# marl-book/codebase

Measured on NVIDIA H100. Metric: env-steps/sec, higher is better.
Workload: dtype f32

## Files before the change

codebase_b200/csrc/dqn.cu:

```cuda
#include "learner.cuh"
#include "dqn_heads.cuh"
#include "retms.cuh"
#include "qmix.cuh"
#include "gru.cuh"
#include <math.h>
#include <stdlib.h>
#include <string.h>
#include <vector>

namespace marl {

__global__ void replay_sample_kernel(uint64_t seed, uint64_t update_idx, int batch, int n_valid, int32_t* idx) {
  const int i = blockIdx.x * blockDim.x + threadIdx.x;
  pdl_wait();
  pdl_launch_dependents();
  if (i >= batch) return;
  const u32x4 b = philox4x32_10((uint32_t)update_idx, (uint32_t)(update_idx >> 32), (uint32_t)(i >> 2), 0u, (uint32_t)seed, (uint32_t)(seed >> 32) ^ kTagSample);
  idx[i] = (int32_t)bounded(pick(b, i & 3), (uint32_t)n_valid);
}

struct ColTdParams {
  const float* q; const float* tq;
  TrajView traj; const int32_t* idx; int B, A; float gamma; int double_q;
  int C, G;
// ... 477 lines not shown
    } else {
      qmix_mix_fn(hl, 0)<<<qb, kQmWarps * 32, qm_smem_bytes(h->ql), st>>>(qp, h->mix_img, h->mix_img_tgt);
    }
    const int want = h->mix_wgrad_tiles ? kQmixChunks : 2 * h->n_sm;
    const int chunk_len = (((Sn + want - 1) / want) + 31) & ~31, chunks = (Sn + chunk_len - 1) / chunk_len;
    if (h->mix_wgrad_tiles) {
      qmix_wgrad_kernel<<<dim3(h->mix_n_tiles, chunks), 256, 0, st>>>(h->mix_rec, Sn, h->mix_tiles, chunk_len, h->mix_part, n);
    } else {
      for (int round = 0; round * kQmMicroPerRound < h->mix_n_micro; ++round)
        qmix_wgrad2_kernel<<<chunks, 256, (size_t)(h->ql.R + 2) * kQmP * sizeof(float), st>>>(h->mix_rec, Sn, h->ql.R, h->mix_micro, h->mix_n_micro, round, chunk_len, h->mix_part, n);
    }
    qmix_reduce_kernel<<<(n + 255) / 256, 256, 0, st>>>(h->mix_part, chunks, n, h->mix_grad, qp.loss_part, qb);
    MARL_CUDA_TRY(cudaGetLastError());
    n_loss_parts += qb;
    tp.td_agent_stride = batch * T;
    return MARL_OK;
  }
  const bool vdn = h->hp.mixer == 1;
  ColTdParams cp; memset(&cp, 0, sizeof(cp));
  cp.q = h->q_all; cp.tq = h->tq; cp.traj = src.traj; cp.idx = src.idx; cp.B = batch; cp.A = h->ns.out;
  cp.gamma = h->hp.gamma; cp.double_q = h->hp.double_q; cp.huber = h->huber; cp.C = vdn ? 1 : h->ns.n_agents; cp.G = vdn ? h->ns.n_agents : 1;
  cp.td = h->td; cp.loss_part = loss_part;
  const int blocks = (cp.C * batch * T + 255) / 256;
  if (h->td_lambda_on) {
    cp.ret = h->ret; cp.chosen = h->chosen; cp.boot = h->boot; cp.stat_per_b = vdn;
    if (h->standardise) { cp.ret_ms = h->ret_ms; cp.n_stat = h->n_stat; }
    col_td_kernel<3><<<blocks, 256, 0, st>>>(cp);
    if (int rc = dqn_td_lambda(h, src, cp.C, cp.G, batch, st)) return rc;
    if (h->standardise) {
      RetMsParams rp; rp.ret = h->ret; rp.part = h->ret_part; rp.ret_ms = h->ret_ms; rp.count = h->ret_count; rp.T = T;
      if (vdn) { rp.N = batch; rp.P = 1; } else { rp.N = cp.C; rp.P = batch; }
      MARL_CUDA_TRY(ret_ms_step(rp, st));
    }
    col_td_kernel<2><<<blocks, 256, 0, st>>>(cp);
  } else if (h->standardise) {
    cp.ret_ms = h->ret_ms; cp.n_stat = h->n_stat; cp.stat_per_b = vdn; cp.ret = h->ret; cp.chosen = h->chosen;
    col_td_kernel<1><<<blocks, 256, 0, st>>>(cp);
    RetMsParams rp; rp.ret = h->ret; rp.part = h->ret_part; rp.ret_ms = h->ret_ms; rp.count = h->ret_count; rp.T = T;
    if (vdn) { rp.N = batch; rp.P = 1; } else { rp.N = cp.C; rp.P = batch; }
    MARL_CUDA_TRY(ret_ms_step(rp, st));
    col_td_kernel<2><<<blocks, 256, 0, st>>>(cp);
  } else {
    col_td_kernel<0><<<blocks, 256, 0, st>>>(cp);
  }
  MARL_CUDA_TRY(cudaGetLastError());
  n_loss_parts += blocks;
  tp.td_agent_stride = vdn ? 0 : batch * T;
  return MARL_OK;
}

static bool dqn_tc_train(const marl_dqn* h) { return !h->rnn && tc_backward_enabled() && h->ns.in < kMaxObsDim && h->image != nullptr; }

static int dqn_tc_prepare(marl_dqn* h, TcBuffers& tb, cudaStream_t st) {
  if (!h->tc_h2) {
    const size_t rows = (size_t)h->ns.n_agents * h->max_batch * (h->max_T + 1), F = sizeof(float);
    if (int rc = alloc_buffers(h, "marl_dqn_update", {{&h->tc_h2, rows * kHidden * F},
                                                      {&h->tc_rec, rows * 32  * F}, {&h->tc_x, rows * ((h->ns.in + 7) / 8 * 8) * F},
                                                      {&h->image_bwd, ((size_t)h->ns.n_nets * tc_bwd_image_bytes() / 4 + 4) * F}}))
      return rc;
  }
  if (!h->image_current || !h->bwd_image_current) {
    if (int rc = launch_pack_weights(h->theta, h->ns.lay, h->ns.n_nets, h->image, st, h->image_bwd)) return rc;
    h->image_current = h->bwd_image_current = true;
  }
  tb.image = h->image; tb.bwd_image = h->image_bwd; tb.h2 = h->tc_h2; tb.rec = h->tc_rec; tb.x = h->tc_x; tb.rows = (size_t)h->ns.n_agents * h->max_batch * (h->max_T + 1);
  return MARL_OK;
}

static int dqn_train_pass(marl_dqn* h, const TrainParams& tp, cudaEvent_t* between, bool& tc, cudaStream_t st) {
  tc = false;
  if (h->rnn) {
    GruBwdParams bp; memset(&bp, 0, sizeof(bp));
    bp.plan = tp.plan; bp.traj = tp.src.traj; bp.idx = tp.src.idx; bp.B = tp.plan.units_per_agent; bp.theta = h->theta; bp.lay = h->gl; bp.save = h->gru_save;
    bp.td = tp.td_ext; bp.td_agent_stride = tp.td_agent_stride; bp.src = tp.src; bp.scratch = h->scratch; bp.scratch_pitch = h->scratch_pitch;
    return launch_gru_backward(bp, st);
  }
  if (!dqn_tc_train(h)) return launch_train(tp, kHeadDqn, st);
  TcBuffers tb;
  if (int rc = dqn_tc_prepare(h, tb, st)) return rc;
  tc = true;
  if (int rc = launch_tc_dqn_forward(tp, tb, nullptr, nullptr, nullptr, st)) return rc;
  if (between) MARL_CUDA_TRY(cudaEventRecord(between[0], st));
  return launch_tc_dqn_backward(tp, tb, st, between ? between[1] : nullptr);
}

static int dqn_fused_pass(marl_dqn* h, const RowPlan& plan, const RowSource& src, int batch, TrainParams& tp, int& n_loss_parts, cudaEvent_t* ev,
                          cudaStream_t st) {
  TcBuffers tb;
  if (int rc = dqn_tc_prepare(h, tb, st)) return rc;
  if (!h->tgt_image_current) {
    if (int rc = launch_pack_weights(h->theta_tgt, h->ns.lay, h->ns.n_nets, h->image_tgt, st)) return rc;
    h->tgt_image_current = true;
  }
  if (ev) MARL_CUDA_TRY(cudaEventRecord(ev[0], st));
  if (int rc = launch_tc_dqn_forward(tp, tb, h->image_tgt, h->tq, dqn_external_head(h) ? h->q_all : nullptr, st)) return rc;
  if (ev) MARL_CUDA_TRY(cudaEventRecord(ev[1], st));
  if (int rc = dqn_td_head(h, plan, src, batch, tp, n_loss_parts, false, st)) return rc;
  if (int rc = launch_tc_dqn_backward(tp, tb, st, ev ? ev[2] : nullptr)) return rc;
  if (ev) { MARL_CUDA_TRY(cudaEventRecord(ev[3], st)); h->ev_used += 1; h->ev_split = true; }
  return MARL_OK;
}

static int dqn_grads(marl_dqn* h, const marl_traj_view* traj, const int32_t* episode_idx, int32_t batch, void* stream, ReduceParams* rp_out) {
  MARL_REQUIRE(h && traj && episode_idx, "marl_dqn_update_grads: NULL argument");
  MARL_REQUIRE(batch >= 1 && batch <= h->max_batch, "marl_dqn_update_grads: batch %d exceeds max_batch %d", batch, h->max_batch);
  MARL_REQUIRE(traj->T >= 1 && traj->T <= h->max_T, "marl_dqn_update_grads: T %d exceeds max_T %d", traj->T, h->max_T);
  MARL_REQUIRE(traj->n_agents == h->ns.n_agents && traj->obs_dim == h->ns.in, "marl_dqn_update_grads: trajectory shape mismatch");
  MARL_REQUIRE(h->hp.mixer != 2 || h->mix != nullptr, "marl_dqn_update: QMIX needs marl_dqn_qmix_init first");
  MARL_REQUIRE(h->hp.mixer == 0 || !h->standardise || batch == h->n_stat, "marl_dqn_update: %s's standardise_returns keeps one statistic per batch entry (the "
               "reference's reshape(-1, B)): batch %d must stay at max_batch %d", h->hp.mixer == 2 ? "QMIX" : "VDN", batch, h->n_stat);
  MARL_CUDA_TRY(cudaSetDevice(h->device));
  cudaStream_t st = (cudaStream_t)stream;
  const RowPlan plan = h->rnn ? make_plan(h->ns, batch, 1, h->n_sm, kGruSeqs) : episode_plan(h->ns, batch, traj->T, h->n_sm);
  const RowSource src = episode_rows(traj, episode_idx, h->ns.n_agents, h->ns.in);
  cudaEvent_t* ev = h->timing && h->ev_used < kTimingPairs ? &h->ev[4 * h->ev_used] : nullptr;
  TrainParams tp; memset(&tp, 0, sizeof(tp));
  tp.plan = plan; tp.src = src; tp.theta = h->theta; tp.lay = h->ns.lay; tp.tq = h->tq;
  tp.gamma = h->hp.gamma; tp.double_q = h->hp.double_q; tp.huber = h->huber; tp.scratch = h->scratch; tp.scratch_pitch = h->scratch_pitch; tp.loss_part = h->loss_part;
// ... 247 lines not shown
```

codebase_b200/csrc/learner.cuh:

```cuda
#pragma once
#include "mlp.cuh"
#include "traj.cuh"
#include <string.h>

namespace marl {

constexpr int kMaxObsDim = 32;
constexpr int kMaxInDim = 128;

struct RowPlan {
  int n_nets;
  int cta_begin[MARL_MAX_AGENTS + 1];
  int slot_begin[MARL_MAX_AGENTS + 1];
  int slot_agent[MARL_MAX_AGENTS];
  int unit_rows;
  int units_per_agent;
};

enum RowMode {
  kRowsDense = 0,
  kRowsEpisode = 1,
  kRowsEpisodeJoint = 2,
  kRowsDenseJoint = 3
};
// ... 190 lines not shown
  p.n_nets = ns.n_nets; p.unit_rows = unit_rows; p.units_per_agent = units_per_agent;
  int s = 0;
  for (int k = 0; k < ns.n_nets; ++k) {
    p.slot_begin[k] = s;
    for (int a = 0; a < ns.n_agents; ++a) if (ns.agent_net[a] == k) p.slot_agent[s++] = a;
  }
  p.slot_begin[ns.n_nets] = s;
  long long total = (long long)ns.n_agents * units_per_agent;
  int c = 0;
  for (int k = 0; k < ns.n_nets; ++k) {
    const long long units = (long long)(p.slot_begin[k + 1] - p.slot_begin[k]) * units_per_agent;
    long long want = (long long)n_cta_max * units / (total > 0 ? total : 1);
    const long long cap = (units + min_units - 1) / min_units;
    if (want > cap) want = cap;
    if (want < 1) want = 1;
    p.cta_begin[k] = c;
    c += (int)want;
  }
  p.cta_begin[ns.n_nets] = c;
  return p;
}

inline RowPlan episode_plan(const NetSet& ns, int episodes, int T, int n_cta_max) {
  const int min_units = (64 + T) / (T + 1) > 0 ? (64 + T) / (T + 1) : 1;
  return make_plan(ns, episodes, T + 1, n_cta_max, min_units);
}

inline RowSource dense_rows(const float* obs, int E, int N, int D, bool joint = false) {
  RowSource s; memset(&s, 0, sizeof(s));
  s.mode = joint ? kRowsDenseJoint : kRowsDense; s.dense = obs; s.E = E; s.N = N; s.D = D;
  if (joint) s.joint = obs;
  return s;
}

inline RowSource episode_rows(const marl_traj_view* t, const int32_t* idx, int N, int D) {
  RowSource s; memset(&s, 0, sizeof(s));
  s.mode = kRowsEpisode; s.traj = traj_view(t); s.idx = idx; s.N = N; s.D = D;
  return s;
}

inline int launch_forward(const NetSet& ns, const RowPlan& plan, const RowSource& src, const float* theta, float* out, cudaStream_t st) {
  FwdParams fp; fp.plan = plan; fp.src = src; fp.theta = theta; fp.lay = ns.lay; fp.out = out;
  return launch_mlp_forward(fp, st);
}

size_t tc_image_bytes();
int tc_forward_init();
size_t tc_bwd_image_bytes();
int launch_pack_weights(const float* theta, const NetLayout& lay, int n_nets, uint8_t* image, cudaStream_t st, uint8_t* bwd_image = nullptr);
int launch_tc_forward(const FwdParams& p, const uint8_t* images, cudaStream_t st);
struct TcBuffers {
  uint8_t* image; uint8_t* bwd_image;
  float* h2;
  float* rec;
  float* x;
  size_t rows;
};
int tc_train_init();
int launch_tc_dqn_forward(const TrainParams& tp, const TcBuffers& buf, const uint8_t* tgt_images, float* tq_out, float* q_out, cudaStream_t st);
int launch_tc_dqn_backward(const TrainParams& tp, const TcBuffers& buf, cudaStream_t st, cudaEvent_t after_dh1 = nullptr);

inline int forward_any(const NetSet& ns, const RowPlan& plan, const RowSource& src, const float* theta, uint8_t* image, float* out, cudaStream_t st,
                       bool image_is_current = false) {
  if (tc_forward_enabled() && image != nullptr && ns.in <= kMaxObsDim && ns.lay.H == kHidden) {
    if (!image_is_current)
      if (int rc = launch_pack_weights(theta, ns.lay, ns.n_nets, image, st)) return rc;
    FwdParams fp; fp.plan = plan; fp.src = src; fp.theta = theta; fp.lay = ns.lay; fp.out = out;
    return launch_tc_forward(fp, image, st);
  }
  return launch_forward(ns, plan, src, theta, out, st);
}

inline int check_mlp_cfg(const marl_mlp_cfg* cfg, const char* who, int max_in) {
  MARL_REQUIRE(cfg != nullptr, "%s: NULL network config", who);
  MARL_REQUIRE(cfg->n_agents >= 1 && cfg->n_agents <= MARL_MAX_AGENTS, "%s: n_agents out of range", who);
  MARL_REQUIRE(cfg->n_nets >= 1 && cfg->n_nets <= cfg->n_agents, "%s: n_nets out of range", who);
  MARL_REQUIRE(cfg->hidden >= 1 && cfg->hidden <= kHidden, "%s: hidden width %d not supported (layers = [H, H], 1 <= H <= %d)", who, cfg->hidden, kHidden);
  MARL_REQUIRE(cfg->in_dim >= 1 && cfg->in_dim <= max_in, "%s: obs dim %d not supported (1..%d)", who, cfg->in_dim, max_in);
  MARL_REQUIRE(cfg->out_dim >= 1 && cfg->out_dim <= kOutPad, "%s: output width %d not supported (1..%d)", who, cfg->out_dim, kOutPad);
  for (int a = 0; a < cfg->n_agents; ++a) MARL_REQUIRE(cfg->agent_net[a] >= 0 && cfg->agent_net[a] < cfg->n_nets, "%s: agent_net[%d] out of range", who, a);
  return MARL_OK;
}

inline NetSet to_netset(const marl_mlp_cfg* cfg) {
  NetSet ns; ns.n_agents = cfg->n_agents; ns.n_nets = cfg->n_nets; ns.in = cfg->in_dim; ns.out = cfg->out_dim;
  memcpy(ns.agent_net, cfg->agent_net, sizeof(int) * MARL_MAX_AGENTS);
  ns.lay = NetLayout::make(cfg->in_dim, cfg->out_dim, cfg->hidden);
  return ns;
}

struct LearnerHandle : BufferOwner {
  int device = 0, n_sm = 148;
  int64_t n_params = 0;
  int scratch_pitch = 0;
  float *theta = nullptr, *theta_tgt = nullptr, *m = nullptr, *v = nullptr, *grad = nullptr, *scratch = nullptr, *loss_part = nullptr;
  int32_t* idx = nullptr;
  uint8_t* image = nullptr;
  marl_optimizer opt = {};
  bool opt_stepped = false;
  int standardise = 0, n_stat = 0; float* ret_ms = nullptr; double *ret_count = nullptr, *ret_part = nullptr;
};

template <typename H, typename HP>
int open_learner(int device, const HP& hp, H** out) {
  if (int rc = check_device(device)) return rc;
  H* h = new H();
  h->hp = hp; h->device = device;
  cudaDeviceProp prop; cudaGetDeviceProperties(&prop, device); h->n_sm = prop.multiProcessorCount;
  h->opt.kind = MARL_OPT_ADAM; h->opt.beta1 = hp.beta1; h->opt.beta2 = hp.beta2; h->opt.eps = hp.eps;
// ... 21 lines not shown
```

codebase_b200/csrc/tc_common.cuh:

```cuda
#pragma once
#include "learner.cuh"
#include <type_traits>

namespace marl {

constexpr int kTcThreads = 256;
constexpr int kWgRows = 64;
constexpr int kPanelBytes = kHidden * 128;
constexpr int kOffW1Hi = 0, kOffW1Lo = kOffW1Hi + kPanelBytes, kOffW2Hi = kOffW1Lo + kPanelBytes, kOffW2Lo = kOffW2Hi + 4 * kPanelBytes;
constexpr int kOffB1 = kOffW2Lo + 4 * kPanelBytes, kOffB2 = kOffB1 + kHidden * 4, kOffB3 = kOffB2 + kHidden * 4;
constexpr int kOffW3F = kOffB3 + kOutPad * 4;
constexpr int kImageBytes = kOffW3F + kOutPad * kHidden * 4;
constexpr int kBwdImageBytes = 8 * kPanelBytes;
static_assert(kOffB1 % 16 == 0 && kOffW3F % 16 == 0 && kImageBytes % 16 == 0, "TMA bulk copies move multiples of 16 bytes");

__device__ __forceinline__ uint32_t smem_u32(const void* p) { return (uint32_t)__cvta_generic_to_shared(p); }
__device__ __forceinline__ float tf32_rn(float x) { return __uint_as_float((__float_as_uint(x) + 0x1000u) & 0xffffe000u); }
__device__ __forceinline__ void tf32_split(float x, float& hi, float& lo) { hi = __uint_as_float(__float_as_uint(x) & 0xffffe000u); lo = x - hi; }
__device__ __forceinline__ void tf32_split_u(float x, uint32_t& hi, uint32_t& lo) { float h, l; tf32_split(x, h, l); hi = __float_as_uint(h); lo = __float_as_uint(l); }

__host__ __device__ __forceinline__ int kperm(int k) { return (k & ~7) | ((k & 1) << 2) | ((k & 7) >> 1); }
__device__ __forceinline__ int panel_offset(int n, int k, int panel_bytes) {
  const int p = k >> 5, c = (k >> 2) & 7, w = k & 3;
  return p * panel_bytes + n * 128 + ((c ^ (n & 7)) << 4) + (w << 2);
// ... 170 lines not shown
    tf32_split_u(v[4 * ks + 0], hi[ks][0], lo[ks][0]); tf32_split_u(v[4 * ks + 2], hi[ks][1], lo[ks][1]);
    tf32_split_u(v[4 * ks + 1], hi[ks][2], lo[ks][2]); tf32_split_u(v[4 * ks + 3], hi[ks][3], lo[ks][3]);
  }
}
__device__ __forceinline__ void head_quad(float (&h)[64], const float* b2, const float* w3f, int out, int quad_lane, float (&q0)[kOutPad], float (&q1)[kOutPad]) {
#pragma unroll
  for (int i = 0; i < 64; i += 2) {
    const float2 bb = *reinterpret_cast<const float2*>(b2 + frag_col(i, quad_lane));
    h[i] = fmaxf(h[i] + bb.x, 0.f); h[i + 1] = fmaxf(h[i + 1] + bb.y, 0.f);
  }
#pragma unroll
  for (int a = 0; a < kOutPad; ++a) {
    float s0 = 0.f, s1 = 0.f;
    if (a < out) {
#pragma unroll
      for (int n = 0; n < 16; ++n) {
        const float2 w = *reinterpret_cast<const float2*>(w3f + a * kHidden + 8 * n + 2 * quad_lane);
        s0 = fmaf(h[4 * n + 1], w.y, fmaf(h[4 * n], w.x, s0));
        s1 = fmaf(h[4 * n + 3], w.y, fmaf(h[4 * n + 2], w.x, s1));
      }
      s0 += __shfl_xor_sync(0xFFFFFFFFu, s0, 1); s1 += __shfl_xor_sync(0xFFFFFFFFu, s1, 1);
      s0 += __shfl_xor_sync(0xFFFFFFFFu, s0, 2); s1 += __shfl_xor_sync(0xFFFFFFFFu, s1, 2);
    }
    q0[a] = s0; q1[a] = s1;
  }
}

template <typename F>
inline int with_k1(int D, F&& f) {
  switch ((D + 7) >> 3) {
    case 1: return f(std::integral_constant<int, 1>());
    case 2: return f(std::integral_constant<int, 2>());
    case 3: return f(std::integral_constant<int, 3>());
    default: return f(std::integral_constant<int, 4>());
  }
}
static_assert(kMaxObsDim == 32, "with_k1 instantiates k-step counts 1 to 4");

constexpr int kRowRec = 32;
constexpr int kRecG = 8, kRecAct = 9, kRecMask1 = 16, kRecMask2 = 20;
__device__ __forceinline__ void frag_masks(const float (&h)[64], uint32_t& m0, uint32_t& m1) {
  m0 = 0; m1 = 0;
#pragma unroll
  for (int i = 0; i < 64; ++i) {
    const uint32_t bit = (h[i] > 0.f ? 1u : 0u) << (((i >> 2) << 1) | (i & 1));
    if (i & 2) m1 |= bit; else m0 |= bit;
  }
}

struct TcTrainParams {
  RowPlan plan; RowSource src; NetLayout lay;
  const uint8_t* images;
  const uint8_t* bwd_images;
  float* h2g; size_t rows;
  float* rec;
  float* xg; int x_pitch;
  const float* tq; const float* td_ext; int td_agent_stride; float gamma; int double_q; float huber;
  float* scratch; int scratch_pitch; float* loss_part;
  const uint8_t* tgt_images; float* tq_out; float* q_out;
};

}
```

codebase_b200/csrc/tc_train.cu:

```cuda
#include "tc_common.cuh"
#include "dqn_heads.cuh"

namespace marl {

__device__ __forceinline__ const float* train_row(const TcTrainParams& p, int net, int vr, size_t& d, int& agent, int& unit, int& off, int& ep) {
  decode_row(p.plan, net, vr, agent, unit, off);
  d = row_index(agent, unit, off, p.plan.units_per_agent, p.plan.unit_rows);
  ep = p.src.idx[unit];
  return p.src.traj.obs_row(ep, agent, off);
}

constexpr int kChunk = 32;
constexpr int kLine = 128;

__device__ __forceinline__ int line_off(int f, int r) { return f * kLine + ((((r >> 2) ^ (f & 7)) & 7) << 4) + ((r & 3) << 2); }
__device__ __forceinline__ void stage_hl(uint8_t* base, int lines, int f, int r, float x) {
  float hi, lo;
  tf32_split(x, hi, lo);
  *reinterpret_cast<float*>(base + line_off(f, r)) = hi;
  *reinterpret_cast<float*>(base + lines * kLine + line_off(f, r)) = lo;
}

TSG_DEFINE(g_ts_fwd)
TSG_GETTER(tsg_fwd, g_ts_fwd)
TSG_DEFINE(g_ts_dh1)
TSG_GETTER(tsg_dh1, g_ts_dh1)
TSG_DEFINE(g_ts_dw)
TSG_GETTER(tsg_dw, g_ts_dw)

__device__ __forceinline__ void store_frag_masks(const float (&v)[64], long long d0, long long d1, int quad_lane, float* rec, int mask) {
  uint32_t m0, m1;
  frag_masks(v, m0, m1);
  if (d0 >= 0) rec[(size_t)d0 * kRowRec + mask + quad_lane] = __uint_as_float(m0);
  if (d1 >= 0) rec[(size_t)d1 * kRowRec + mask + quad_lane] = __uint_as_float(m1);
}
__device__ __forceinline__ void store_frag_fm(float* dst, size_t rows, const float (&v)[64], long long d0, long long d1, int quad_lane, float* rec, int mask) {
#pragma unroll
  for (int i = 0; i < 64; ++i) {
    const long long d = (i & 2) ? d1 : d0;
    if (d >= 0) dst[(size_t)frag_col(i, quad_lane) * rows + (size_t)d] = v[i];
  }
  store_frag_masks(v, d0, d1, quad_lane, rec, mask);
}

constexpr int kTgtW1 = (kImageBytes + 1023) / 1024 * 1024;
constexpr int kTgtB1 = kTgtW1 + (kOffW2Hi - kOffW1Hi);
constexpr int kFwdBar = kTgtB1 + (kImageBytes - kOffB1);
constexpr int kFwdTrainSmem = kFwdBar + 4 * 8 + 1024;
static_assert(kOffW1Hi == 0 && kTgtW1 % 1024 == 0 && kFwdBar % 16 == 0 && kFwdTrainSmem <= 227 * 1024,
              "training forward: 1024-byte aligned target W1 panels, online image and target operands within the shared memory of one SM");

template <int K1>
__global__ void __launch_bounds__(kTcThreads, 1) tc_dqn_fwd_kernel(TcTrainParams p) {
  extern __shared__ uint8_t smem_raw[];
  uint8_t* smem = align_smem_1024(smem_raw);
  uint64_t* bar = reinterpret_cast<uint64_t*>(smem + kFwdBar);
  const int t = threadIdx.x, wg = t >> 7, wq = (t >> 5) & 3, lane = t & 31, g = lane >> 2, tq = lane & 3;
  int net, row_begin, row_end;
  cta_rows(p.plan, net, row_begin, row_end);
  if (row_begin >= row_end) { pdl_wait(); return; }
  TSG(g_ts_fwd, 0);
  const bool tgt = p.tgt_images != nullptr;
  if (t == 0) { for (int i = 0; i < 4; ++i) mbar_init(bar + i, 1); fence_mbar_init(); }
  __syncthreads();
  pdl_wait();
  pdl_launch_dependents();
  const uint32_t sb = smem_u32(smem);
  if (t == 0) {
    tma_forward_image(sb, p.images + (size_t)net * kImageBytes, bar);
    if (tgt) {
      const uint8_t* timg = p.tgt_images + (size_t)net * kImageBytes;
      mbar_expect_tx(bar + 2, (uint32_t)((kOffW2Hi - kOffW1Hi) + (kImageBytes - kOffB1)));
      tma_image_range(sb + kTgtW1, timg, kOffW1Hi, kOffW2Hi, bar + 2);
      tma_image_range(sb + kTgtB1 - kOffB1, timg, kOffB1, kImageBytes, bar + 2);
    }
  }
  const float* b1 = reinterpret_cast<const float*>(smem + kOffB1);
  const float* b2 = reinterpret_cast<const float*>(smem + kOffB2);
  const float* b3 = reinterpret_cast<const float*>(smem + kOffB3);
  const float* w3f = reinterpret_cast<const float*>(smem + kOffW3F);
  const int D = p.src.D, A = p.lay.out;
  auto online_w2_done = [&]() {
    if (wg == 0) {
      named_bar_sync(1, kTcThreads);
      if (t == 0) {
        mbar_expect_tx(bar + 3, (uint32_t)(kOffB1 - kOffW2Hi));
        tma_image_range(sb, p.tgt_images + (size_t)net * kImageBytes, kOffW2Hi, kOffB1, bar + 3);
      }
    } else {
      named_bar_arrive(1, kTcThreads);
    }
  };
  bool first = true;
  for (int vr0 = row_begin + kWgRows * wg; vr0 < row_end; vr0 += kTileRows) {
    const int r0 = vr0 + 16 * wq + g, r1 = r0 + 8;
    size_t d0u = 0, d1u = 0;
    int agent, unit, off, ep;
    const float* s0 = r0 < row_end ? train_row(p, net, r0, d0u, agent, unit, off, ep) : nullptr;
    const float* s1 = r1 < row_end ? train_row(p, net, r1, d1u, agent, unit, off, ep) : nullptr;
    const long long d0 = s0 ? (long long)d0u : -1, d1 = s1 ? (long long)d1u : -1;
    float acc[64];
    {
      float x[kMaxObsDim / 8][4];
      load_x_frag(s0, s1, D, tq, x);
#pragma unroll
      for (int ks = 0; ks < kMaxObsDim / 8; ++ks) {
        const int c = 8 * ks + 2 * tq;
        if (ks < K1) {
          if (d0 >= 0) *reinterpret_cast<float2*>(p.xg + (size_t)d0 * p.x_pitch + c) = make_float2(x[ks][0], x[ks][2]);
          if (d1 >= 0) *reinterpret_cast<float2*>(p.xg + (size_t)d1 * p.x_pitch + c) = make_float2(x[ks][1], x[ks][3]);
        }
      }
      if (first) mbar_wait(bar, 0);
      layer1_tile<K1>(acc, x, sb + kOffW1Hi, b1, tq);
    }
    store_frag_masks(acc, d0, d1, tq, p.rec, kRecMask1);
    {
      uint32_t hi[16][4], lo[16][4];
      frag_to_a(acc, hi, lo);
      if (first) { mbar_wait(bar + 1, 0); first = false; }
#pragma unroll
      for (int i = 0; i < 64; ++i) acc[i] = 0.f;
      layer_rs<16>(acc, hi, lo, sb + kOffW2Hi, sb + kOffW2Lo, 16);
    }
    if (tgt && vr0 + kTileRows >= row_end) online_w2_done();
    float q0[kOutPad], q1[kOutPad];
    head_quad(acc, b2, w3f, A, tq, q0, q1);
    store_frag_fm(p.h2g, p.rows, acc, d0, d1, tq, p.rec, kRecMask2);
    const long long d = tq == 0 ? d0 : d1;
    if (tq < 2 && d >= 0) {
      float* o = p.rec + (size_t)d * kRowRec;
#pragma unroll
      for (int a = 0; a < kOutPad; ++a) {
        const float v = a < A ? (tq == 0 ? q0[a] : q1[a]) + b3[a] : 0.f;
        o[a] = v;
        if (p.q_out != nullptr && a < A) p.q_out[(size_t)d * A + a] = v;
      }
    }
  }
  if (!tgt) { TSG(g_ts_fwd, 31); return; }
  if (row_begin + kWgRows * wg >= row_end) online_w2_done();
  TSG(g_ts_fwd, 16);
  const float* tb1 = reinterpret_cast<const float*>(smem + kTgtB1);
  const float* tb2 = reinterpret_cast<const float*>(smem + kTgtB1 + (kOffB2 - kOffB1));
  const float* tb3 = reinterpret_cast<const float*>(smem + kTgtB1 + (kOffB3 - kOffB1));
  const float* tw3f = reinterpret_cast<const float*>(smem + kTgtB1 + (kOffW3F - kOffB1));
  const int n_tiles = (row_end - row_begin + kWgRows - 1) / kWgRows, n_mine = wg == 0 ? n_tiles / 2 : (n_tiles + 1) / 2;
  first = true;
  for (int i = 0; i < n_mine; ++i) {
    const bool moved = wg + 2 * i >= n_tiles;
    const int vr0 = row_begin + kWgRows * (moved ? n_tiles - 1 : wg + 2 * i);
    if (moved && first) mbar_wait(bar + 3, 0);
    const int r0 = vr0 + 16 * wq + g, r1 = r0 + 8;
    long long d0 = -1, d1 = -1;
    {
      int agent, unit, off;
      if (r0 < row_end) { decode_row(p.plan, net, r0, agent, unit, off); d0 = (long long)row_index(agent, unit, off, p.plan.units_per_agent, p.plan.unit_rows); }
      if (r1 < row_end) { decode_row(p.plan, net, r1, agent, unit, off); d1 = (long long)row_index(agent, unit, off, p.plan.units_per_agent, p.plan.unit_rows); }
    }
    float acc[64];
    {
      float x[kMaxObsDim / 8][4];
#pragma unroll
      for (int ks = 0; ks < kMaxObsDim / 8; ++ks) {
        const int c = 8 * ks + 2 * tq;
        float2 v0 = make_float2(0.f, 0.f), v1 = make_float2(0.f, 0.f);
        if (ks < K1) {
          if (d0 >= 0) v0 = *reinterpret_cast<const float2*>(p.xg + (size_t)d0 * p.x_pitch + c);
          if (d1 >= 0) v1 = *reinterpret_cast<const float2*>(p.xg + (size_t)d1 * p.x_pitch + c);
        }
        x[ks][0] = v0.x; x[ks][1] = v1.x; x[ks][2] = v0.y; x[ks][3] = v1.y;
      }
      if (first) mbar_wait(bar + 2, 0);
      layer1_tile<K1>(acc, x, sb + kTgtW1, tb1, tq);
    }
    {
      uint32_t hi[16][4], lo[16][4];
      frag_to_a(acc, hi, lo);
      if (first) { mbar_wait(bar + 3, 0); first = false; }
#pragma unroll
      for (int i = 0; i < 64; ++i) acc[i] = 0.f;
      layer_rs<16>(acc, hi, lo, sb + kOffW2Hi, sb + kOffW2Lo, 16);
    }
    float q0[kOutPad], q1[kOutPad];
    head_quad(acc, tb2, tw3f, A, tq, q0, q1);
    const long long d = tq == 0 ? d0 : d1;
    if (tq < 2 && d >= 0) {
      float* o = p.tq_out + (size_t)d * A;
#pragma unroll
      for (int a = 0; a < kOutPad; ++a)
        if (a < A) o[a] = (tq == 0 ? q0[a] : q1[a]) + tb3[a];
// ... 136 lines not shown
      const int k = (i >> 1) & 1, bit = ((i >> 2) << 1) | (i & 1);
      v[i] = ((mh2[k] >> bit) & 1u) ? gr[k] * w3f[act[k] * kHidden + frag_col(i, tq)] : 0.f;
      m1 |= (uint64_t)((mh1[k] >> bit) & 1u) << i;
    }
#pragma unroll
    for (int i = 0; i < 64; ++i) acc[i] = 0.f;
    if (vr0 < row_end) {
      uint32_t hi[16][4], lo[16][4];
      frag_to_a(v, hi, lo);
      layer_rs<16>(acc, hi, lo, sb, sb + 4 * kPanelBytes, 16);
    }
#pragma unroll
    for (int k = 0; k < 2; ++k)
#pragma unroll
      for (int m = 0; m < kMaxObsDim / 4; ++m) {
        const int f = tq + 4 * m;
        xv[k][m] = (d[k] >= 0 && f < D) ? p.xg[(size_t)d[k] * p.x_pitch + f] : 0.f;
      }
    const long long dr = tq == 0 ? d[0] : d[1];
    if (tq < 2 && dr >= 0) {
      float* rp = p.rec + (size_t)dr * kRowRec;
      rp[kRecG] = tq == 0 ? gr[0] : gr[1]; rp[kRecAct] = __int_as_float(tq == 0 ? act[0] : act[1]);
    }
    dw1_phase(0, c0, row_begin, row_end, D, smem, sb, acc, m1, xv, acc1);
  }
  {
    const int c_last = (row_end - 1 - row_begin) / kTileRows * (kTileRows / kChunk);
    if (row_begin + (c_last + 2) * kChunk < row_end) dw1_phase(1, c_last + 2, row_begin, row_end, D, smem, sb, acc, m1, xv, acc1);
  }
  wg_wait<0>();
  fence_regs(acc1);
  TSG(g_ts_dh1, 30);
  {
    const NetLayout& L = p.lay;
    float* gs = p.scratch + (size_t)blockIdx.x * p.scratch_pitch;
#pragma unroll
    for (int i = 0; i < 16; ++i) {
      const int m = wg * kWgRows + 16 * wq + g + ((i & 2) ? 8 : 0), n = frag_col(i, tq);
      if (n < D) gs[L.w1 + m * D + n] = acc1[i];
      else if (n == D) gs[L.b1 + m] = acc1[i];
    }
  }
  red[t] = st0; red[kTcThreads + t] = st1;
  __syncthreads();
  for (int s = kTcThreads / 2; s > 0; s >>= 1) {
    if (t < s) { red[t] += red[t + s]; red[kTcThreads + t] += red[kTcThreads + t + s]; }
    __syncthreads();
  }
  if (t < 4) p.loss_part[4 * blockIdx.x + t] = t < 2 ? red[t * kTcThreads] : 0.f;
  TSG(g_ts_dh1, 31);
}

constexpr int kB2Bytes = 2 * 136 * kLine;
constexpr int kW3Pitch = kHidden + 1;
constexpr int kSA2 = 0, kSB2 = kSA2 + 2 * 128 * kLine, kSA3 = kSB2 + 2 * kB2Bytes, kSB3 = kSA3 + 2 * 128 * kLine, kSW1 = kSB3 + 2 * 8 * kLine;
constexpr int kSW3 = kSW1 + (kOffW2Hi - kOffW1Hi);
constexpr int kSB1 = kSW3 + (kOutPad * kW3Pitch * 4 + 15) / 16 * 16, kSBar = kSB1 + kHidden * 4;
constexpr int kDwSmem = kSBar + 64 + 1024;
static_assert(kSB2 % 1024 == 0 && kB2Bytes % 1024 == 0 && kSA3 % 1024 == 0 && kSB3 % 1024 == 0 && kSW1 % 1024 == 0 && kSB1 % 16 == 0 &&
              kDwSmem <= 227 * 1024, "weight-gradient staging: 1024-byte aligned operands within the shared memory of one SM");

__device__ __forceinline__ const float* xg_row(const TcTrainParams& p, int net, int vr) {
  int agent, unit, off;
  decode_row(p.plan, net, vr, agent, unit, off);
  return p.xg + row_index(agent, unit, off, p.plan.units_per_agent, p.plan.unit_rows) * (size_t)p.x_pitch;
}

template <int K1>
__global__ void __launch_bounds__(kTcThreads, 1) tc_dw_kernel(TcTrainParams p) {
  extern __shared__ uint8_t smem_raw[];
  uint8_t* smem = align_smem_1024(smem_raw);
  const float* w3f = reinterpret_cast<const float*>(smem + kSW3);
  const float* b1 = reinterpret_cast<const float*>(smem + kSB1);
  uint64_t* bar = reinterpret_cast<uint64_t*>(smem + kSBar);
  const int t = threadIdx.x, warp = t >> 5, wg = t >> 7, wq = (t >> 5) & 3, lane = t & 31, g = lane >> 2, tq = lane & 3;
  int net, row_begin, row_end;
  cta_rows(p.plan, net, row_begin, row_end);
  float* gs = p.scratch + (size_t)blockIdx.x * p.scratch_pitch;
  pdl_wait();
  pdl_launch_dependents();
  if (row_begin >= row_end) {
    for (int i = t; i < p.lay.P; i += kTcThreads) gs[i] = 0.f;
    return;
  }
  TSG(g_ts_dw, 0);
  const uint32_t sb = smem_u32(smem);
  if (t == 0) {
    mbar_init(bar, 1); fence_mbar_init();
    const uint8_t* img = p.images + (size_t)net * kImageBytes;
    mbar_expect_tx(bar, (uint32_t)((kOffW2Hi - kOffW1Hi) + kHidden * 4));
    tma_image_range(sb + kSW1 - kOffW1Hi, img, kOffW1Hi, kOffW2Hi, bar);
    tma_bulk_g2s(sb + kSB1, img + kOffB1, kHidden * 4, bar);
  }
  const int A = p.lay.out, D = p.src.D;
  for (int i = t; i < 2 * 8 * kChunk; i += kTcThreads) {
    const int b = i / (8 * kChunk), f = 128 + (i / kChunk) % 8, r = i % kChunk;
    stage_hl(smem + kSB2 + b * kB2Bytes, 136, f, r, f == 128 ? 1.f : 0.f);
  }
  {
    const float* w3src = reinterpret_cast<const float*>(p.images + (size_t)net * kImageBytes + kOffW3F);
    for (int i = t; i < kOutPad * kHidden; i += kTcThreads) reinterpret_cast<float*>(smem + kSW3)[(i / kHidden) * kW3Pitch + i % kHidden] = w3src[i];
  }
  __syncthreads();
  TSG(g_ts_dw, 1);
  float acc2[68], acc3[4];
#pragma unroll
  for (int i = 0; i < 68; ++i) acc2[i] = 0.f;
#pragma unroll
  for (int i = 0; i < 4; ++i) acc3[i] = 0.f;
  float db3 = 0.f;
  bool first = true;
  const int n_chunks = (row_end - row_begin + kChunk - 1) / kChunk;
  int c = 0;
  do {
    TSG(g_ts_dw, 2 + c);
    const int vr = row_begin + c * kChunk + lane;
    float h2v[16], gr = 0.f;
    int act = 0;
    {
      long long d = -1;
      if (vr < row_end) {
        int agent, unit, off;
        decode_row(p.plan, net, vr, agent, unit, off);
        d = (long long)row_index(agent, unit, off, p.plan.units_per_agent, p.plan.unit_rows);
        const float* rp = p.rec + (size_t)d * kRowRec;
        gr = rp[kRecG]; act = __float_as_int(rp[kRecAct]);
      }
#pragma unroll
      for (int i = 0; i < 16; ++i) h2v[i] = d >= 0 ? p.h2g[(size_t)(warp + 8 * i) * p.rows + (size_t)d] : 0.f;
    }
    const bool rebuild = (c & 1) == 0 && wg == ((c >> 1) & 1);
    const int r0 = row_begin + c * kChunk + 16 * wq + g, r1 = r0 + 8;
    float x[kMaxObsDim / 8][4], h1[64];
    if (rebuild) load_x_frag(r0 < row_end ? xg_row(p, net, r0) : nullptr, r1 < row_end ? xg_row(p, net, r1) : nullptr, D, tq, x);
    wg_wait<0>();
    fence_regs(acc2); fence_regs(acc3);
    if (rebuild) {
      if (first) { mbar_wait(bar, 0); first = false; }
      layer1_tile<K1>(h1, x, sb + kSW1, b1, tq);
    }
    __syncthreads();
#pragma unroll
    for (int i = 0; i < 16; ++i) {
      const int j = warp + 8 * i;
      const float dh2 = h2v[i] > 0.f ? gr * w3f[act * kW3Pitch + j] : 0.f;
      stage_hl(smem + kSA2, 128, j, lane, dh2);
      stage_hl(smem + kSA3, 128, j, lane, h2v[i]);
    }
    {
      const float dq = act == warp ? gr : 0.f;
      stage_hl(smem + kSB3, 8, warp, lane, dq);
      float s = dq;
#pragma unroll
      for (int o = 16; o > 0; o >>= 1) s += __shfl_xor_sync(0xFFFFFFFFu, s, o);
      db3 += s;
    }
    if (rebuild) {
      uint8_t* b2 = smem + kSB2 + (wq >> 1) * kB2Bytes;
      const int cr = 16 * (wq & 1) + g;
#pragma unroll
      for (int i = 0; i < 64; ++i) stage_hl(b2, 136, frag_col(i, tq), cr + ((i & 2) ? 8 : 0), (((i & 2) ? r1 : r0) < row_end) ? h1[i] : 0.f);
    }
    asm volatile("fence.proxy.async.shared::cta;" ::: "memory");
    __syncthreads();
    wg_fence();
    const uint32_t m_off = (uint32_t)(wg * kWgRows * kLine), b2_off = (uint32_t)(kSB2 + (c & 1) * kB2Bytes);
#pragma unroll
    for (int term = 0; term < 3; ++term) {
      const uint32_t ah = term == 0 ? 1u : 0u, bh = term == 1 ? 1u : 0u;
#pragma unroll
      for (int ks = 0; ks < kChunk / 8; ++ks) {
        const uint32_t ko = (uint32_t)(ks * 32);
        wgmma_ss_n136(acc2, sw128_desc(sb + kSA2 + ah * 128 * kLine + m_off + ko), sw128_desc(sb + b2_off + bh * 136 * kLine + ko), 1u);
        wgmma_ss_n8(acc3, sw128_desc(sb + kSA3 + ah * 128 * kLine + m_off + ko), sw128_desc(sb + kSB3 + bh * 8 * kLine + ko), 1u);
      }
    }
    wg_commit();
  } while (++c < n_chunks);
  wg_wait<0>();
  fence_regs(acc2); fence_regs(acc3);
  TSG(g_ts_dw, 30);
  const NetLayout& L = p.lay;
#pragma unroll
  for (int i = 0; i < 64; i += 2) {
    const int m = wg * kWgRows + 16 * wq + g + ((i & 2) ? 8 : 0), n = frag_col(i, tq);
    *reinterpret_cast<float2*>(gs + L.w2 + m * kHidden + n) = make_float2(acc2[i], acc2[i + 1]);
  }
#pragma unroll
  for (int i = 64; i < 68; ++i) {
    const int m = wg * kWgRows + 16 * wq + g + ((i & 2) ? 8 : 0), n = frag_col(i, tq);
    if (n == kHidden) gs[L.b2 + m] = acc2[i];
  }
#pragma unroll
  for (int i = 0; i < 4; ++i) {
    const int m = wg * kWgRows + 16 * wq + g + ((i & 2) ? 8 : 0), n = frag_col(i, tq);
    if (n < A) gs[L.w3 + n * kHidden + m] = acc3[i];
  }
  if (lane == 0 && warp < A) gs[L.b3 + warp] = db3;
  TSG(g_ts_dw, 31);
}


int tc_train_init() {
  MARL_CUDA_TRY(cudaFuncSetAttribute(tc_dh1_kernel, cudaFuncAttributeMaxDynamicSharedMemorySize, kDh1Smem));
  for (int D = 1; D <= kMaxObsDim; D += 8)
    if (int rc = with_k1(D, [](auto k1) {
          MARL_CUDA_TRY(cudaFuncSetAttribute(tc_dqn_fwd_kernel<decltype(k1)::value>, cudaFuncAttributeMaxDynamicSharedMemorySize, kFwdTrainSmem));
          MARL_CUDA_TRY(cudaFuncSetAttribute(tc_dw_kernel<decltype(k1)::value>, cudaFuncAttributeMaxDynamicSharedMemorySize, kDwSmem));
          return MARL_OK;
        }))
      return rc;
  return MARL_OK;
}

static TcTrainParams tc_params(const TrainParams& tp, const TcBuffers& buf) {
  TcTrainParams p; memset(&p, 0, sizeof(p));
  p.plan = tp.plan; p.src = tp.src; p.lay = tp.lay; p.images = buf.image; p.bwd_images = buf.bwd_image;
  p.h2g = buf.h2; p.rec = buf.rec; p.xg = buf.x; p.x_pitch = 8 * ((tp.src.D + 7) / 8); p.rows = buf.rows;
  p.tq = tp.tq; p.td_ext = tp.td_ext; p.td_agent_stride = tp.td_agent_stride; p.gamma = tp.gamma; p.double_q = tp.double_q; p.huber = tp.huber;
  p.scratch = tp.scratch; p.scratch_pitch = tp.scratch_pitch; p.loss_part = tp.loss_part;
  return p;
}

int launch_tc_dqn_forward(const TrainParams& tp, const TcBuffers& buf, const uint8_t* tgt_images, float* tq_out, float* q_out, cudaStream_t st) {
  MARL_REQUIRE(tp.lay.in < kMaxObsDim, "tensor-core backward: observation width %d needs a spare column for the bias trick (max %d)", tp.lay.in, kMaxObsDim - 1);
  MARL_REQUIRE(tp.src.mode == 1, "tensor-core backward: rows must be gathered from the trajectory store (mode %d)", tp.src.mode);
  MARL_REQUIRE(tgt_images == nullptr || tq_out != nullptr, "tensor-core training forward: target images without an output buffer");
  TcTrainParams p = tc_params(tp, buf);
  p.tgt_images = tgt_images; p.tq_out = tq_out; p.q_out = q_out;
  return with_k1(tp.src.D, [&](auto k1) {
    MARL_CUDA_TRY(launch_pdl(tc_dqn_fwd_kernel<decltype(k1)::value>, dim3(tp.plan.cta_begin[tp.plan.n_nets]), dim3(kTcThreads), kFwdTrainSmem, st, p));
    return MARL_OK;
  });
}

int launch_tc_dqn_backward(const TrainParams& tp, const TcBuffers& buf, cudaStream_t st, cudaEvent_t after_dh1) {
  const TcTrainParams p = tc_params(tp, buf);
  const int grid = tp.plan.cta_begin[tp.plan.n_nets];
  MARL_CUDA_TRY(launch_pdl(tc_dh1_kernel, dim3(grid), dim3(kTcThreads), kDh1Smem, st, p));
  if (after_dh1) MARL_CUDA_TRY(cudaEventRecord(after_dh1, st));
  return with_k1(tp.src.D, [&](auto k1) {
    MARL_CUDA_TRY(launch_pdl(tc_dw_kernel<decltype(k1)::value>, dim3(grid), dim3(kTcThreads), kDwSmem, st, p));
    return MARL_OK;
  });
}

}
```

Measured before the change: 125,800.

## Store forward H2 activations in per-CTA fragment-ordered slabs for backward reuse

The forward training kernel previously scattered the hidden-layer-2 activations feature-major into a global array with strided per-element stores. The backward dW kernel then re-gathered them with strided loads. Both kernels now use per-CTA tile slabs written and read as coalesced float4 in MMA fragment order. The dW kernel shuffles gradient and action values across lanes to stage them, and the W3 pitch is padded for aligned float2 reads. This needs a larger, slab-padded H2 allocation with a capacity check, and adds timestamp probes in the forward loop.

Measured after the change: 136,200 (median of 6 runs). 8.2% higher.

```diff
diff --git a/codebase_b200/csrc/dqn.cu b/codebase_b200/csrc/dqn.cu
--- a/codebase_b200/csrc/dqn.cu
+++ b/codebase_b200/csrc/dqn.cu
@@ -553,9 +553,10 @@
 static bool dqn_tc_train(const marl_dqn* h) { return !h->rnn && tc_backward_enabled() && h->ns.in < kMaxObsDim && h->image != nullptr; }
 
 static int dqn_tc_prepare(marl_dqn* h, TcBuffers& tb, cudaStream_t st) {
+  const size_t rows = (size_t)h->ns.n_agents * h->max_batch * (h->max_T + 1), h2_tiles = (rows + 63) / 64 + (size_t)h->n_sm;
   if (!h->tc_h2) {
-    const size_t rows = (size_t)h->ns.n_agents * h->max_batch * (h->max_T + 1), F = sizeof(float);
-    if (int rc = alloc_buffers(h, "marl_dqn_update", {{&h->tc_h2, rows * kHidden * F},
+    const size_t F = sizeof(float);
+    if (int rc = alloc_buffers(h, "marl_dqn_update", {{&h->tc_h2, h2_tiles * 64 * kHidden * F},
                                                       {&h->tc_rec, rows * 32  * F}, {&h->tc_x, rows * ((h->ns.in + 7) / 8 * 8) * F},
                                                       {&h->image_bwd, ((size_t)h->ns.n_nets * tc_bwd_image_bytes() / 4 + 4) * F}}))
       return rc;
@@ -564,7 +565,7 @@
     if (int rc = launch_pack_weights(h->theta, h->ns.lay, h->ns.n_nets, h->image, st, h->image_bwd)) return rc;
     h->image_current = h->bwd_image_current = true;
   }
-  tb.image = h->image; tb.bwd_image = h->image_bwd; tb.h2 = h->tc_h2; tb.rec = h->tc_rec; tb.x = h->tc_x; tb.rows = (size_t)h->ns.n_agents * h->max_batch * (h->max_T + 1);
+  tb.image = h->image; tb.bwd_image = h->image_bwd; tb.h2 = h->tc_h2; tb.h2_tiles = h2_tiles; tb.rec = h->tc_rec; tb.x = h->tc_x;
   return MARL_OK;
 }
 
diff --git a/codebase_b200/csrc/learner.cuh b/codebase_b200/csrc/learner.cuh
--- a/codebase_b200/csrc/learner.cuh
+++ b/codebase_b200/csrc/learner.cuh
@@ -266,9 +266,9 @@
 struct TcBuffers {
   uint8_t* image; uint8_t* bwd_image;
   float* h2;
+  size_t h2_tiles;
   float* rec;
   float* x;
-  size_t rows;
 };
 int tc_train_init();
 int launch_tc_dqn_forward(const TrainParams& tp, const TcBuffers& buf, const uint8_t* tgt_images, float* tq_out, float* q_out, cudaStream_t st);
diff --git a/codebase_b200/csrc/tc_common.cuh b/codebase_b200/csrc/tc_common.cuh
--- a/codebase_b200/csrc/tc_common.cuh
+++ b/codebase_b200/csrc/tc_common.cuh
@@ -246,7 +246,7 @@
   RowPlan plan; RowSource src; NetLayout lay;
   const uint8_t* images;
   const uint8_t* bwd_images;
-  float* h2g; size_t rows;
+  float4* h2s;
   float* rec;
   float* xg; int x_pitch;
   const float* tq; const float* td_ext; int td_agent_stride; float gamma; int double_q; float huber;
diff --git a/codebase_b200/csrc/tc_train.cu b/codebase_b200/csrc/tc_train.cu
--- a/codebase_b200/csrc/tc_train.cu
+++ b/codebase_b200/csrc/tc_train.cu
@@ -34,14 +34,10 @@
   if (d0 >= 0) rec[(size_t)d0 * kRowRec + mask + quad_lane] = __uint_as_float(m0);
   if (d1 >= 0) rec[(size_t)d1 * kRowRec + mask + quad_lane] = __uint_as_float(m1);
 }
-__device__ __forceinline__ void store_frag_fm(float* dst, size_t rows, const float (&v)[64], long long d0, long long d1, int quad_lane, float* rec, int mask) {
-#pragma unroll
-  for (int i = 0; i < 64; ++i) {
-    const long long d = (i & 2) ? d1 : d0;
-    if (d >= 0) dst[(size_t)frag_col(i, quad_lane) * rows + (size_t)d] = v[i];
-  }
-  store_frag_masks(v, d0, d1, quad_lane, rec, mask);
-}
+__device__ __forceinline__ size_t h2_slab(const RowPlan& p, int net, int row_begin) {
+  return (size_t)(((long long)p.slot_begin[net] * p.units_per_agent * p.unit_rows + row_begin) / kWgRows) + blockIdx.x;
+}
+constexpr int kH2TileF4 = 16 * 128;
 
 constexpr int kTgtW1 = (kImageBytes + 1023) / 1024 * 1024;
 constexpr int kTgtB1 = kTgtW1 + (kOffW2Hi - kOffW1Hi);
@@ -92,7 +88,10 @@
     }
   };
   bool first = true;
-  for (int vr0 = row_begin + kWgRows * wg; vr0 < row_end; vr0 += kTileRows) {
+  float4* const h2s = p.h2s + h2_slab(p.plan, net, row_begin) * kH2TileF4 + (t & 127);
+  int it = 0;
+  for (int vr0 = row_begin + kWgRows * wg; vr0 < row_end; vr0 += kTileRows, ++it) {
+    if (it < 5) TSG(g_ts_fwd, 1 + 3 * it);
     const int r0 = vr0 + 16 * wq + g, r1 = r0 + 8;
     size_t d0u = 0, d1u = 0;
     int agent, unit, off, ep;
@@ -123,10 +122,16 @@
       for (int i = 0; i < 64; ++i) acc[i] = 0.f;
       layer_rs<16>(acc, hi, lo, sb + kOffW2Hi, sb + kOffW2Lo, 16);
     }
+    if (it < 5) TSG(g_ts_fwd, 2 + 3 * it);
     if (tgt && vr0 + kTileRows >= row_end) online_w2_done();
     float q0[kOutPad], q1[kOutPad];
     head_quad(acc, b2, w3f, A, tq, q0, q1);
-    store_frag_fm(p.h2g, p.rows, acc, d0, d1, tq, p.rec, kRecMask2);
+    {
+      float4* h2 = h2s + (size_t)((vr0 - row_begin) / kWgRows) * kH2TileF4;
+#pragma unroll
+      for (int n = 0; n < 16; ++n) h2[n * 128] = make_float4(acc[4 * n], acc[4 * n + 1], acc[4 * n + 2], acc[4 * n + 3]);
+    }
+    store_frag_masks(acc, d0, d1, tq, p.rec, kRecMask2);
     const long long d = tq == 0 ? d0 : d1;
     if (tq < 2 && d >= 0) {
       float* o = p.rec + (size_t)d * kRowRec;
@@ -137,6 +142,7 @@
         if (p.q_out != nullptr && a < A) p.q_out[(size_t)d * A + a] = v;
       }
     }
+    if (it < 5) TSG(g_ts_fwd, 3 + 3 * it);
   }
   if (!tgt) { TSG(g_ts_fwd, 31); return; }
   if (row_begin + kWgRows * wg >= row_end) online_w2_done();
@@ -379,7 +385,7 @@
 }
 
 constexpr int kB2Bytes = 2 * 136 * kLine;
-constexpr int kW3Pitch = kHidden + 1;
+constexpr int kW3Pitch = kHidden + 8;
 constexpr int kSA2 = 0, kSB2 = kSA2 + 2 * 128 * kLine, kSA3 = kSB2 + 2 * kB2Bytes, kSB3 = kSA3 + 2 * 128 * kLine, kSW1 = kSB3 + 2 * 8 * kLine;
 constexpr int kSW3 = kSW1 + (kOffW2Hi - kOffW1Hi);
 constexpr int kSB1 = kSW3 + (kOutPad * kW3Pitch * 4 + 15) / 16 * 16, kSBar = kSB1 + kHidden * 4;
@@ -438,23 +444,25 @@
   float db3 = 0.f;
   bool first = true;
   const int n_chunks = (row_end - row_begin + kChunk - 1) / kChunk;
+  const float4* const h2s = p.h2s + h2_slab(p.plan, net, row_begin) * kH2TileF4 + 4 * (t >> 6) * 128 + (t & 63);
+  const int cr = 16 * (warp & 1) + g;
   int c = 0;
   do {
     TSG(g_ts_dw, 2 + c);
     const int vr = row_begin + c * kChunk + lane;
-    float h2v[16], gr = 0.f;
+    float gr = 0.f;
     int act = 0;
-    {
-      long long d = -1;
-      if (vr < row_end) {
-        int agent, unit, off;
-        decode_row(p.plan, net, vr, agent, unit, off);
-        d = (long long)row_index(agent, unit, off, p.plan.units_per_agent, p.plan.unit_rows);
-        const float* rp = p.rec + (size_t)d * kRowRec;
-        gr = rp[kRecG]; act = __float_as_int(rp[kRecAct]);
-      }
-#pragma unroll
-      for (int i = 0; i < 16; ++i) h2v[i] = d >= 0 ? p.h2g[(size_t)(warp + 8 * i) * p.rows + (size_t)d] : 0.f;
+    if (vr < row_end) {
+      int agent, unit, off;
+      decode_row(p.plan, net, vr, agent, unit, off);
+      const float* rp = p.rec + row_index(agent, unit, off, p.plan.units_per_agent, p.plan.unit_rows) * kRowRec;
+      gr = rp[kRecG]; act = __float_as_int(rp[kRecAct]);
+    }
+    float4 h2q[4];
+    {
+      const float4* src = h2s + (size_t)(c >> 1) * kH2TileF4 + 64 * (c & 1);
+#pragma unroll
+      for (int m = 0; m < 4; ++m) h2q[m] = src[m * 128];
     }
     const bool rebuild = (c & 1) == 0 && wg == ((c >> 1) & 1);
     const int r0 = row_begin + c * kChunk + 16 * wq + g, r1 = r0 + 8;
@@ -468,11 +476,21 @@
     }
     __syncthreads();
 #pragma unroll
-    for (int i = 0; i < 16; ++i) {
-      const int j = warp + 8 * i;
-      const float dh2 = h2v[i] > 0.f ? gr * w3f[act * kW3Pitch + j] : 0.f;
-      stage_hl(smem + kSA2, 128, j, lane, dh2);
-      stage_hl(smem + kSA3, 128, j, lane, h2v[i]);
+    for (int k = 0; k < 2; ++k) {
+      const int r = cr + 8 * k;
+      const bool live = row_begin + c * kChunk + r < row_end;
+      const float g_r = __shfl_sync(0xFFFFFFFFu, gr, r);
+      const int act_r = __shfl_sync(0xFFFFFFFFu, act, r);
+#pragma unroll
+      for (int m = 0; m < 4; ++m) {
+        const int j = 8 * (4 * (t >> 6) + m) + 2 * tq;
+        const float2 w = *reinterpret_cast<const float2*>(w3f + act_r * kW3Pitch + j);
+        const float h0 = live ? (k ? h2q[m].z : h2q[m].x) : 0.f, h1v = live ? (k ? h2q[m].w : h2q[m].y) : 0.f;
+        stage_hl(smem + kSA2, 128, j, r, h0 > 0.f ? g_r * w.x : 0.f);
+        stage_hl(smem + kSA2, 128, j + 1, r, h1v > 0.f ? g_r * w.y : 0.f);
+        stage_hl(smem + kSA3, 128, j, r, h0);
+        stage_hl(smem + kSA3, 128, j + 1, r, h1v);
+      }
     }
     {
       const float dq = act == warp ? gr : 0.f;
@@ -543,7 +561,7 @@
 static TcTrainParams tc_params(const TrainParams& tp, const TcBuffers& buf) {
   TcTrainParams p; memset(&p, 0, sizeof(p));
   p.plan = tp.plan; p.src = tp.src; p.lay = tp.lay; p.images = buf.image; p.bwd_images = buf.bwd_image;
-  p.h2g = buf.h2; p.rec = buf.rec; p.xg = buf.x; p.x_pitch = 8 * ((tp.src.D + 7) / 8); p.rows = buf.rows;
+  p.h2s = reinterpret_cast<float4*>(buf.h2); p.rec = buf.rec; p.xg = buf.x; p.x_pitch = 8 * ((tp.src.D + 7) / 8);
   p.tq = tp.tq; p.td_ext = tp.td_ext; p.td_agent_stride = tp.td_agent_stride; p.gamma = tp.gamma; p.double_q = tp.double_q; p.huber = tp.huber;
   p.scratch = tp.scratch; p.scratch_pitch = tp.scratch_pitch; p.loss_part = tp.loss_part;
   return p;
@@ -553,6 +571,11 @@
   MARL_REQUIRE(tp.lay.in < kMaxObsDim, "tensor-core backward: observation width %d needs a spare column for the bias trick (max %d)", tp.lay.in, kMaxObsDim - 1);
   MARL_REQUIRE(tp.src.mode == 1, "tensor-core backward: rows must be gathered from the trajectory store (mode %d)", tp.src.mode);
   MARL_REQUIRE(tgt_images == nullptr || tq_out != nullptr, "tensor-core training forward: target images without an output buffer");
+  {
+    const RowPlan& pl = tp.plan;
+    const size_t tiles = ((size_t)pl.slot_begin[pl.n_nets] * pl.units_per_agent * pl.unit_rows + kWgRows - 1) / kWgRows + pl.cta_begin[pl.n_nets];
+    MARL_REQUIRE(tiles <= buf.h2_tiles, "tensor-core training forward: the H2 slabs need %zu tiles, %zu allocated", tiles, buf.h2_tiles);
+  }
   TcTrainParams p = tc_params(tp, buf);
   p.tgt_images = tgt_images; p.tq_out = tq_out; p.q_out = q_out;
   return with_k1(tp.src.D, [&](auto k1) {
```
